# mindspore-lab/minddet

Hardware: AMD Instinct MI355X
Metric: images/sec, Faster R-CNN R50-FPN inference, COCO-shaped 1333x800 (padded 800x1344) (higher is better)
Workload: dtype bf16; 1 GPU; faster_rcnn_r50_fpn_800x1344 (BASELINE.json configs[2]); batch_per_gpu=120, streams=2, global_batch=120, parallelism=dp1 (image sharding + all_gather of detections), weights=random init, seed 7

## Files before the change

### minddet_amd/graphs.py

```python
import math
import os

import numpy as np
import torch

from . import det_ops, nn_ops
from .registry import BACKBONES, DETECTORS, HEADS, NECKS, READERS, ROI_HEAD, build_backbone, build_head, build_neck, build_roi_head


RPN_OVERLAP = os.environ.get("MD_RPN_OVERLAP", "1") == "1"
FUSE_BLOCKS = os.environ.get("MD_FUSE_BLOCKS", "1") == "1"
FUSE_DUAL = os.environ.get("MD_FUSE_DUAL", "1") == "1"
RPN_FUSED_HEAD = os.environ.get("MD_RPN_FUSED", "1") == "1"


class SplitForward:

    def __init__(self, model, streams=2):
        self.model, self.n = model, int(streams)
        self._streams = None
        self._primed = set()

    def __call__(self, images, prepare=None, **kw):
        ins = images if isinstance(images, (tuple, list)) else (images,)
        B = ins[0].shape[0]
        if self.n <= 1 or B < self.n or B % self.n or kw.get("return_aux"):
            return self.model.forward(images if prepare is None else prepare(*ins), **kw)
        dev = ins[0].device
        if self._streams is None or self._streams[0].device != dev:
            self._streams = [torch.cuda.Stream(device=dev) for _ in range(self.n)]
            self._primed = set()
        step = B // self.n

        def part(i):
            p = [t[i * step:(i + 1) * step] for t in ins]
            return p[0] if prepare is None else prepare(*p)

        cur = torch.cuda.current_stream(dev)
        key = (Module.generation, step, prepare is not None) + tuple(ins[0].shape[1:])
        if key not in self._primed:
            self.model.forward(part(0), **kw)
            self._primed.add(key)
        outs = []
        for i, st in enumerate(self._streams):
            st.wait_stream(cur)
            with torch.cuda.stream(st):
                outs.append(self.model.forward(part(i), **kw))
        for st in self._streams:
            cur.wait_stream(st)
        res = []
        for k in range(len(outs[0])):
            ts = [o[k] for o in outs]
            for t in ts:
                t.record_stream(cur)
            res.append(torch.cat(ts, 0))
        return tuple(res)


def _split_forward_of(model, test_cfg):
    model.streams = int((test_cfg or {}).get("streams", 1))
    model.forward_split = SplitForward(model, model.streams)


class ParamInit:

    def __init__(self, seed=7):
        self.rng = np.random.default_rng(seed)

    def conv(self, cout, cin, k, std=None):
        std = math.sqrt(2.0 / (k * k * cout)) if std is None else std
        return torch.from_numpy(self.rng.normal(0.0, std, (cout, cin, k, k)).astype(np.float32))

    def bn(self, c, eps=1e-5):
        return (torch.ones(c), torch.zeros(c), torch.from_numpy(self.rng.normal(0, 0.1, c).astype(np.float32)),
                torch.from_numpy(self.rng.uniform(0.5, 1.5, c).astype(np.float32)), eps)

    def bias(self, c, value=None, std=0.01):
        if value is not None:
            return torch.full((c,), float(value))
        return torch.from_numpy(self.rng.normal(0, std, c).astype(np.float32))


class Module:
    generation = 0

    def children(self):
        return []

    def modules(self):
        ch = self.children()
        return [m for c in ch for m in c.modules()] if ch else [self]

    conv_modules = modules

    def to(self, device):
        for c in self.children():
            c.to(device)
        self._derive(device)
        self._consts = {}
        Module.generation += 1
        return self

    def _derive(self, device):
        pass

    def const(self, key, build):
        if key not in self._consts:
            self._consts[key] = build()
        return self._consts[key]


def _segments(B, n, device):
    return torch.arange(0, (B + 1) * n, n, dtype=torch.int32, device=device)


def _image_hw(images):
    border = nn_ops.STEM_PAD_LO + nn_ops.STEM_PAD_HI if images.shape[3] == 4 else 0
    return images.shape[1] - border, images.shape[2] - border


class ConvModule(Module):

    def __init__(self, init, cin, cout, k, stride=1, pad=0, bn=True, relu=True, bias=False, bn_eps=1e-5, std=None,
                 bias_value=None, act=None):
        self.act = act if act is not None else ("relu" if relu else None)
        relu = self.act == "relu"
        self.cin, self.cout, self.k, self.stride, self.pad, self.relu = cin, cout, k, stride, pad, relu
        self.weight = init.conv(cout, cin, k, std)
        self.bn = init.bn(cout, bn_eps) if bn else None
        self.bias = init.bias(cout, bias_value) if bias else None
        self.packed = None

    def _derive(self, device):
        self.packed = nn_ops.pack_conv(self.weight, bias=self.bias, bn=self.bn, stride=self.stride, pad=self.pad,
                                       relu=self.act).to(device)

    def __call__(self, x, residual=None, out=None, c_off=0, x_c_off=None, res_c_off=None):
        return nn_ops.conv2d(x, self.packed, residual=residual, out=out, c_off=c_off, x_c_off=x_c_off, res_c_off=res_c_off)

    def macs(self, ho, wo):
        return ho * wo * self.cout * self.cin * self.k * self.k


def merged_conv(mods, device):
    m0 = mods[0]
    if any((m.cin, m.k, m.stride, m.pad, m.act, m.bn is None, m.bias is None) != (m0.cin, m0.k, m0.stride, m0.pad, m0.act, m0.bn is None, m0.bias is None)
           for m in mods):
        raise ValueError("merged_conv: the convs must share input, geometry and activation")
    w = torch.cat([m.weight for m in mods], 0)
    bn = None if m0.bn is None else tuple(torch.cat([torch.as_tensor(m.bn[i]) for m in mods]) for i in range(4)) + (m0.bn[4],)
    bias = None if m0.bias is None else torch.cat([m.bias for m in mods])
    return nn_ops.pack_conv(w, bias=bias, bn=bn, stride=m0.stride, pad=m0.pad, relu=m0.act).to(device)


class BasicBlock(Module):
    expansion = 1

    def __init__(self, init, inplanes, planes, stride=1, downsample=None):
        self.conv1 = ConvModule(init, inplanes, planes, 3, stride, 1)
        self.conv2 = ConvModule(init, planes, planes, 3, 1, 1, relu=True)
        self.downsample = downsample

    def children(self):
        return [self.conv1, self.conv2] + ([self.downsample] if self.downsample else [])

    def __call__(self, x):
        residual = self.downsample(x) if self.downsample is not None else x
        out = self.conv1(x)
        return self.conv2(out, residual=residual)


class Bottleneck(Module):
    expansion = 4

    def __init__(self, init, inplanes, planes, stride=1, downsample=None):
        self.conv1 = ConvModule(init, inplanes, planes, 1)
        self.conv2 = ConvModule(init, planes, planes, 3, stride, 1)
        self.conv3 = ConvModule(init, planes, planes * 4, 1, relu=True)
        self.downsample = downsample
        self._fused = self._dual = None

    def children(self):
        return [self.conv1, self.conv2, self.conv3] + ([self.downsample] if self.downsample else [])

    def _derive(self, device):
        pd = self.downsample.packed if self.downsample is not None else None
        self._fused = nn_ops.pack_bottleneck(self.conv1.packed, self.conv2.packed, self.conv3.packed, pd)
        self._dual = nn_ops.pack_dual(self.conv3.packed, pd) if pd is not None else None

    def __call__(self, x):
        if FUSE_BLOCKS and self._fused is not None:
            res = self.downsample(x) if (self.downsample is not None and self._fused.wd is None) else None
            return nn_ops.bottleneck(x, self._fused, residual=res)
        if FUSE_DUAL and self._dual is not None:
            return nn_ops.conv1x1_dual(self.conv2(self.conv1(x)), x, self._dual)
        residual = self.downsample(x) if self.downsample is not None else x
        return self.conv3(self.conv2(self.conv1(x)), residual=residual)


@BACKBONES.register_module
class ResNet(Module):
    SETTINGS = {18: (BasicBlock, [2, 2, 2, 2]), 34: (BasicBlock, [3, 4, 6, 3]), 50: (Bottleneck, [3, 4, 6, 3]),
                101: (Bottleneck, [3, 4, 23, 3])}

    def __init__(self, depth=50, base_width=64, seed=7, init=None, layers=None):
        block, default_layers = self.SETTINGS[depth]
        layers = layers or default_layers
        init = init or ParamInit(seed)
        self.block, self.inplanes = block, base_width
        self.conv1 = ConvModule(init, 3, base_width, 7, 2, 3)
        self.stages = []
        for i, n in enumerate(layers):
            self.stages.append(self._make_layer(init, block, base_width * (2 ** i), n, 1 if i == 0 else 2))
        self.out_channels = [base_width * (2 ** i) * block.expansion for i in range(4)]

    def _make_layer(self, init, block, planes, blocks, stride):
        downsample = None
        if stride != 1 or self.inplanes != planes * block.expansion:
            downsample = ConvModule(init, self.inplanes, planes * block.expansion, 1, stride, 0, relu=False)
        layers = [block(init, self.inplanes, planes, stride, downsample)]
        self.inplanes = planes * block.expansion
        for _ in range(1, blocks):
            layers.append(block(init, self.inplanes, planes))
        return layers

    def children(self):
        return [self.conv1] + [b for st in self.stages for b in st]

    def _derive(self, device):
        self.stem = None
        if self.conv1.cout == 64 and self.conv1.relu:
            self.stem = nn_ops.pack_stem(self.conv1.weight, bn=self.conv1.bn, bias=self.conv1.bias).to(device)

    def __call__(self, x):
        if x.shape[3] == 4:
            if self.stem is None:
                raise nn_ops._lib.MindDetHipError("ResNet: stem-layout input needs the 64-channel ReLU stem")
            x = nn_ops.stem_pool(x, self.stem)
        else:
            x = self.conv1(x)
            x = nn_ops.maxpool2d(x, 3, 2, 1, zero_pad=True)
        outs = []
        for st in self.stages:
            for b in st:
                x = b(x)
            outs.append(x)
        return tuple(outs)


@NECKS.register_module
class FPN(Module):

    def __init__(self, in_channels, out_channels=256, num_outs=5, seed=11, init=None):
        init = init or ParamInit(seed)
        self.lateral = [ConvModule(init, c, out_channels, 1, bn=False, relu=False, bias=True) for c in in_channels]
        self.output = [ConvModule(init, out_channels, out_channels, 3, 1, 1, bn=False, relu=False, bias=True)
                       for _ in in_channels]
        self.num_outs = num_outs

    def children(self):
        return self.lateral + self.output

    def __call__(self, feats):
        lats = [None] * len(feats)
        lats[-1] = self.lateral[-1](feats[-1])
        for i in range(len(feats) - 2, -1, -1):
            h, w = feats[i].shape[1], feats[i].shape[2]
            top = lats[i + 1]
            if top.shape[1] == (h + 1) // 2 and top.shape[2] == (w + 1) // 2:
                lats[i] = nn_ops.conv2d(feats[i], self.lateral[i].packed, residual=top, res_upsample=True)
            else:
                lats[i] = nn_ops.upsample_add(self.lateral[i](feats[i]), top)
        outs = [o(l) for o, l in zip(self.output, lats)]
        while len(outs) < self.num_outs:
            outs.append(nn_ops.maxpool2d(outs[-1], 1, 2, 0, zero_pad=False))
        return outs


@HEADS.register_module
class RPNHead(Module):

    def __init__(self, in_channels=256, feat_channels=256, strides=(4, 8, 16, 32, 64), scale=8.0,
                 ratios=(0.5, 1.0, 2.0), nms_pre=1000, max_per_img=1000, nms_thr=0.7, seed=13, init=None):
        init = init or ParamInit(seed)
        self.A = len(ratios)
        self.conv = ConvModule(init, in_channels, feat_channels, 3, 1, 1, bn=False, relu=True, bias=True, std=0.01)
        self.out = ConvModule(init, feat_channels, 5 * self.A, 1, bn=False, relu=False, bias=True, std=0.01)
        self.strides, self.scale, self.ratios = tuple(strides), scale, tuple(ratios)
        self.nms_pre, self.max_per_img, self.nms_thr = nms_pre, max_per_img, nms_thr

    def children(self):
        return [self.conv, self.out]

    def _static(self, feats, img_hw):
        B, dev = feats[0].shape[0], feats[0].device
        sizes = tuple((f.shape[1], f.shape[2]) for f in feats)

        def build():
            anchors = det_ops.fpn_anchors(sizes, self.strides, self.scale, self.ratios, device=dev)
            per, offs, o = [], [], 0
            for (h, w) in sizes:
                n = h * w * self.A
                per.append(anchors[o:o + n])
                offs.append(_segments(B, n, dev))
                o += n
            return dict(anchors=per, seg=offs, merged_seg=_segments(B, len(sizes) * self.nms_pre, dev))

        return self.const((B, sizes, img_hw), build)

    def __call__(self, feats, img_hw):
        st = self._static(feats, img_hw)
        B, L, k, A = feats[0].shape[0], len(feats), self.nms_pre, self.A
        dev = feats[0].device
        boxes = torch.empty((L, B, k, 4), dtype=torch.float32, device=dev)
        scores = torch.empty((L, B, k), dtype=torch.float32, device=dev)
        counts = torch.empty((L, B), dtype=torch.int32, device=dev)
        heads = []
        main = torch.cuda.current_stream(dev) if RPN_OVERLAP else None
        side = self.const("side", lambda: torch.cuda.Stream(dev)) if RPN_OVERLAP else None
        keep_alive = []
        if RPN_OVERLAP:
            for t in (boxes, scores, counts):
                t.record_stream(side)
        try:
            for l, f in enumerate(feats):
                if RPN_FUSED_HEAD and self.conv.cout == 256 and self.out.packed.cout == 16 and self.conv.relu:
                    head = nn_ops.conv2d_head(f, self.conv.packed, self.out.packed)
                else:
                    head = self.out(self.conv(f))
                heads.append(head)

                def select(l=l, f=f, head=head):
                    logits = nn_ops.slice_cast(head, 0, A)
                    _, idx, cnt = det_ops.topk_segmented(logits, st["seg"][l], k, out_cnt=counts[l],
                                                         max_segment=f.shape[1] * f.shape[2] * A)
                    det_ops.rpn_decode(head, st["anchors"][l], idx, cnt, A, img_hw, out_boxes=boxes[l], out_scores=scores[l])
                    keep_alive.append((logits, idx, cnt))

                if RPN_OVERLAP:
                    head.record_stream(side)
                    ev = torch.cuda.Event()
                    ev.record(main)
                    with torch.cuda.stream(side):
                        side.wait_event(ev)
                        select()
                else:
                    select()
        finally:
            if RPN_OVERLAP:
                main.wait_stream(side)
        keep, _, _ = det_ops.nms_aligned(boxes.view(L * B, k, 4), self.nms_thr, mode=det_ops.NMS_MODE_STRICT,
                                         count=counts.view(-1))
        mboxes, mscores = det_ops.rpn_merge(boxes, scores, keep.view(L, B, k))
        topv, topi, cnt = det_ops.topk_segmented(mscores, st["merged_seg"], self.max_per_img, max_segment=L * k)
        rois, roi_scores = det_ops.make_rois(mboxes, topv, topi, cnt)
        return rois, roi_scores, cnt, dict(heads=heads, boxes=boxes, scores=scores, counts=counts, keep=keep,
                                           mboxes=mboxes, mscores=mscores)


@ROI_HEAD.register_module
class StandardRoIHead(Module):

    def __init__(self, in_channels=256, fc_channels=1024, num_classes=80, roi_size=7, sampling_ratio=2,
                 featmap_strides=(4, 8, 16, 32), score_thr=0.05, nms_thr=0.5, max_per_img=100, nms_pre=2048,
                 seed=17, init=None):
        init = init or ParamInit(seed)
        self.nc, self.P, self.C = num_classes, roi_size, in_channels
        k_in = in_channels * roi_size * roi_size
        self.fc1 = ConvModule(init, k_in, fc_channels, 1, bn=False, relu=True, bias=True, std=math.sqrt(2.0 / k_in))
        self.fc2 = ConvModule(init, fc_channels, fc_channels, 1, bn=False, relu=True, bias=True,
                              std=math.sqrt(2.0 / fc_channels))
        self.reg_offset = (num_classes + 1 + 7) // 8 * 8
        n_out = self.reg_offset + 4 * num_classes
        self.fc_out = ConvModule(init, fc_channels, n_out, 1, bn=False, relu=False, bias=True, std=0.01)
        self.fc_out.weight[num_classes + 1:self.reg_offset] = 0
        self.fc_out.bias[num_classes + 1:self.reg_offset] = 0
        self.fc_out.weight[:num_classes + 1] *= 20.0
        self.strides, self.sampling = tuple(featmap_strides), sampling_ratio
        self.score_thr, self.nms_thr, self.max_per_img, self.nms_pre = score_thr, nms_thr, max_per_img, nms_pre
        self.prefix_status = det_ops.PrefixStatus()

    def children(self):
        return [self.fc1, self.fc2, self.fc_out]

    def __call__(self, feats, rois, roi_cnt, img_hw):
        B = feats[0].shape[0]
        R = rois.shape[0]
        post = R // B
        dev = rois.device
        pooled = det_ops.roi_align(list(feats[:len(self.strides)]), rois, self.P, [1.0 / s for s in self.strides],
                                   self.sampling, True)
        x = nn_ops.linear(pooled.view(R, self.P * self.P * self.C), self.fc1.packed)
        x = nn_ops.linear(x, self.fc2.packed)
        cls_reg = nn_ops.linear(x, self.fc_out.packed)
        cand = det_ops.rcnn_scores(cls_reg, roi_cnt, self.nc, self.score_thr)
        seg = self.const((B, post), lambda: _segments(B, post * self.nc, dev))
        sv, si, sc = det_ops.topk_segmented(cand, seg, self.nms_pre, max_segment=post * self.nc)
        boxes, labels = det_ops.rcnn_decode_selected(cls_reg, rois, si, sc, self.nc, self.reg_offset, img_hw)
        keep, kidx, num = det_ops.nms_aligned(boxes, self.nms_thr, mode=det_ops.NMS_MODE_STRICT, count=sc, group=labels,
                                              max_output=self.max_per_img)
        dets, count = det_ops.pack_detections(boxes, sv, labels, kidx, num, self.max_per_img, sel_cnt=sc,
                                              status=self.prefix_status.tensor(B, dev))
        return dets, count, dict(pooled=pooled, cls_reg=cls_reg, cand=cand, sel_scores=sv, sel_idx=si, sel_cnt=sc,
                                 boxes=boxes, labels=labels, keep=keep)


@DETECTORS.register_module
class FasterRCNN(Module):

    def __init__(self, backbone, neck, rpn_head, roi_head, train_cfg=None, test_cfg=None):
        self.backbone = build_backbone(backbone)
        neck = dict(neck)
        neck.setdefault("in_channels", self.backbone.out_channels)
        self.neck = build_neck(neck)
        self.rpn_head = build_head(rpn_head)
        self.roi_head = build_roi_head(roi_head)
        self.test_cfg = test_cfg
        _split_forward_of(self, test_cfg)

    def children(self):
        return [self.backbone, self.neck, self.rpn_head, self.roi_head]

    @property
    def prefix_status(self):
        return self.roi_head.prefix_status

    def extract_feat(self, images):
        return self.neck(self.backbone(images))

    def forward(self, images, return_aux=False):
        img_hw = _image_hw(images)
        feats = self.extract_feat(images)
        rois, roi_scores, roi_cnt, aux_rpn = self.rpn_head(feats, img_hw)
        dets, count, aux_roi = self.roi_head(feats, rois, roi_cnt, img_hw)
        if return_aux:
            return dets, count, dict(feats=feats, rois=rois, roi_scores=roi_scores, roi_cnt=roi_cnt, rpn=aux_rpn, roi=aux_roi)
        return dets, count

    __call__ = forward

    def macs_per_image(self, h, w, num_rois=None):
        total, hh, ww = 0, h, w
        bb = self.backbone

        def out_hw(m, hh, ww):
            return (hh + 2 * m.pad - m.k) // m.stride + 1, (ww + 2 * m.pad - m.k) // m.stride + 1

        hh, ww = out_hw(bb.conv1, hh, ww)
        total += bb.conv1.macs(hh, ww)
        hh, ww = (hh + 2 - 3) // 2 + 1, (ww + 2 - 3) // 2 + 1
        sizes = []
        for st in bb.stages:
            for b in st:
                h_in, w_in = hh, ww
                for m in b.modules():
                    if m is b.downsample:
                        ho, wo = out_hw(m, h_in, w_in)
                        total += m.macs(ho, wo)
                    else:
                        hh, ww = out_hw(m, hh, ww)
                        total += m.macs(hh, ww)
            sizes.append((hh, ww))
        for l, (a, b_) in zip(self.neck.lateral, sizes):
            total += l.macs(a, b_)
        for o, (a, b_) in zip(self.neck.output, sizes):
            total += o.macs(a, b_)
        lv = list(sizes)
        while len(lv) < self.neck.num_outs:
            lv.append(((lv[-1][0] - 1) // 2 + 1, (lv[-1][1] - 1) // 2 + 1))
        for (a, b_) in lv:
            total += self.rpn_head.conv.macs(a, b_) + self.rpn_head.out.macs(a, b_)
        r = num_rois if num_rois is not None else self.rpn_head.max_per_img
        for m in self.roi_head.modules():
            total += r * m.cout * m.cin
        return total


class DeconvModule(Module):

    def __init__(self, init, cin, cout, k, stride, pad, bn=True, relu=True, bn_eps=1e-5):
        self.cin, self.cout, self.k, self.stride, self.pad, self.relu = cin, cout, k, stride, pad, relu
        std = math.sqrt(2.0 / (k * k * cout))
        self.weight_t = torch.from_numpy(init.rng.normal(0.0, std, (cin, cout, k, k)).astype(np.float32))
        self.bn = init.bn(cout, bn_eps) if bn else None
        self.packed = None

    def _derive(self, device):
        self.packed = nn_ops.pack_conv_transpose(self.weight_t, bn=self.bn, stride=self.stride, pad=self.pad,
                                                 relu=self.relu).to(device)

    def __call__(self, x, out=None, c_off=0):
        return nn_ops.conv_transpose2d(x, self.packed, out=out, c_off=c_off)


@ROI_HEAD.register_module
class FCNMaskHead(Module):

    def __init__(self, in_channels=256, conv_channels=256, num_convs=4, num_classes=80, roi_size=14, sampling_ratio=2,
                 featmap_strides=(4, 8, 16, 32), seed=19, init=None):
        init = init or ParamInit(seed)
        self.nc, self.P, self.C = num_classes, roi_size, in_channels
        self.convs = []
        cin = in_channels
        for _ in range(num_convs):
            self.convs.append(ConvModule(init, cin, conv_channels, 3, 1, 1, bn=False, relu=True, bias=True))
            cin = conv_channels
        self.upsample = DeconvModule(init, cin, conv_channels, 2, 2, 0, bn=False, relu=True)
        self.logits = ConvModule(init, conv_channels, num_classes, 1, bn=False, relu=False, bias=True, std=0.05)
        self.strides, self.sampling = tuple(featmap_strides), sampling_ratio

    def children(self):
        return self.convs + [self.upsample, self.logits]

    def __call__(self, feats, dets):
        B, D = dets.shape[0], dets.shape[1]
        rois = det_ops.dets_to_rois(dets)
        x = det_ops.roi_align(list(feats[:len(self.strides)]), rois, self.P, [1.0 / s for s in self.strides], self.sampling, True)
        for m in self.convs:
            x = m(x)
        x = self.logits(self.upsample(x))
        masks = det_ops.mask_select(x, dets.view(B * D, 6), self.nc)
        return masks.view(B, D, 2 * self.P, 2 * self.P), dict(rois=rois, logits=x)


@DETECTORS.register_module
class MaskRCNN(FasterRCNN):

    def __init__(self, backbone, neck, rpn_head, roi_head, mask_head, train_cfg=None, test_cfg=None):
        super().__init__(backbone, neck, rpn_head, roi_head, train_cfg, test_cfg)
        self.mask_head = build_roi_head(mask_head)
        tc = test_cfg or {}
        self.paste = bool(tc.get("paste_masks", False))
        self.mask_thr = float(tc.get("mask_thr_binary", 0.5))

    def children(self):
        return super().children() + [self.mask_head]

    def forward(self, images, return_aux=False, paste=None):
        dets, count, aux = FasterRCNN.forward(self, images, return_aux=True)
        masks, aux_mask = self.mask_head(aux["feats"], dets)
        out = (dets, count, masks)
        if self.paste if paste is None else paste:
            out = out + (det_ops.paste_masks(masks, dets, _image_hw(images), self.mask_thr, bits=True),)
        if return_aux:
            aux["mask"] = aux_mask
            return out + (aux,)
        return out

# ... 808 lines not shown
```

### minddet_amd/nn_ops.py

```python
import ctypes

import torch

from . import _lib


class ConvTune(ctypes.Structure):
    _fields_ = [("chunk_limit", ctypes.c_int32), ("stream_rounds", ctypes.c_int32), ("stream_wgs_per_cu", ctypes.c_int32),
                ("stream_cache_bits", ctypes.c_int32), ("pers_min_k", ctypes.c_int32), ("dual_pp_min_k", ctypes.c_int32)]


class _ConvAttrs(ctypes.Structure):
    _fields_ = [("kh", ctypes.c_int32), ("kw", ctypes.c_int32), ("stride", ctypes.c_int32), ("pad", ctypes.c_int32),
                ("relu", ctypes.c_int32), ("variant", ctypes.c_int32), ("adv", ctypes.c_int32), ("pad_top", ctypes.c_int32),
                ("pad_left", ctypes.c_int32), ("sub_h", ctypes.c_int32), ("sub_w", ctypes.c_int32),
                ("out_stride", ctypes.c_int32), ("out_off_y", ctypes.c_int32), ("out_off_x", ctypes.c_int32),
                ("c_off", ctypes.c_int32), ("cout", ctypes.c_int32), ("res_upsample", ctypes.c_int32), ("korder", ctypes.c_int32),
                ("x_c_off", ctypes.c_int32), ("x_cin", ctypes.c_int32), ("res_slice", ctypes.c_int32), ("res_c_off", ctypes.c_int32),
                ("reserved0", ctypes.c_int32), ("tune", ConvTune)]


def cout_tile(cout):
    return 128 if cout > 64 else (64 if cout > 32 else 32)


def _round_up(x, m):
    return (x + m - 1) // m * m


KORDER_DEFAULT = 0


ACT_CODES = {None: 0, False: 0, True: 1, "relu": 1, "silu": 2, 0: 0, 1: 1, 2: 2}


class _PackedWB:

    def to(self, device):
        self.w, self.bias = self.w.to(device), self.bias.to(device)
        return self


class PackedConv(_PackedWB):

    def __init__(self, w, bias, cin, cout, kh, kw, stride, pad, relu):
        self.w, self.bias = w, bias
        self.cin, self.cout, self.kh, self.kw = cin, cout, kh, kw
        self.stride, self.pad, self.relu = stride, pad, relu

    def flops(self, n, ho, wo):
        return 2 * n * ho * wo * self.cout * self.cin_real * self.kh * self.kw

    cin_real = 0


def _fold_bn(weight, bias, bn):
    weight = weight.detach().to(torch.float32)
    if bn is None:
        return weight, (bias.detach().to(torch.float32) if bias is not None else torch.zeros(weight.shape[0]))
    gamma, beta, mean, var, eps = bn
    scale = gamma.to(torch.float32) / torch.sqrt(var.to(torch.float32) + eps)
    b = beta.to(torch.float32) - mean.to(torch.float32) * scale
    if bias is not None:
        b = b + bias.to(torch.float32) * scale
    return weight * scale.view(-1, 1, 1, 1), b


def pack_conv(weight, bias=None, bn=None, stride=1, pad=0, relu=False, cin_pad_to=8, cout_pad_to=8, korder=None):
    cout, cin, kh, kw = weight.shape
    weight, b = _fold_bn(weight, bias, bn)
    cin_p = _round_up(cin, cin_pad_to)
    cout_o = _round_up(cout, cout_pad_to)
    cout_p = _round_up(cout_o, cout_tile(cout_o))
    k_real = kh * kw * cin_p
    k_pad = _round_up(k_real, 64)
    wp = torch.zeros((cout_p, kh, kw, cin_p), dtype=torch.float32, device=weight.device)
    wp[:cout, :, :, :cin] = weight.permute(0, 2, 3, 1)
    if korder is None:
        halo = kh == 3 and kw == 3 and stride == 1 and pad == 1 and cin_p % 64 == 0 and cout_o >= 64
        korder = 1 if halo else KORDER_DEFAULT
    if korder == 1:
        wp = wp.reshape(cout_p, kh, kw, cin_p // 64, 64).permute(0, 3, 1, 2, 4).contiguous()
    wk = torch.zeros((cout_p, k_pad), dtype=torch.float32, device=weight.device)
    wk[:, :k_real] = wp.reshape(cout_p, k_real)
    bp = torch.zeros((cout_p,), dtype=torch.float32, device=weight.device)
    bp[:cout] = b.to(weight.device)
    pc = PackedConv(wk.to(torch.bfloat16).contiguous(), bp.contiguous(), cin_p, cout_o, kh, kw, stride, pad, ACT_CODES[relu])
    pc.cin_real = cin
    pc.korder = korder
    return pc


def conv_out_hw(h, w, pc):
    return (h + 2 * pc.pad - pc.kh) // pc.stride + 1, (w + 2 * pc.pad - pc.kw) // pc.stride + 1


import os as _os
TUNE = ConvTune(dual_pp_min_k=int(_os.environ.get("MD_DUAL_PP_MIN_K", "0")), pers_min_k=int(_os.environ.get("MD_PERS_MIN_K", "0")))


def conv2d(x, pc, residual=None, relu=None, out=None, variant=None, c_off=0, res_upsample=False, x_c_off=None, res_c_off=None, tune=None):
    n, h, w, c = x.shape
    if x_c_off is None and c != pc.cin:
        raise _lib.MindDetHipError(f"conv2d: input has {c} channels, layer packed for {pc.cin}")
    ho, wo = conv_out_hw(h, w, pc)
    if out is None:
        out = torch.empty((n, ho, wo, pc.cout), dtype=torch.bfloat16, device=x.device)
    attrs = _ConvAttrs(pc.kh, pc.kw, pc.stride, pc.pad, int(pc.relu if relu is None else relu),
                       int(variant or 0))
    attrs.korder = getattr(pc, "korder", 0)
    attrs.tune = TUNE if tune is None else tune
    attrs.res_upsample = int(bool(res_upsample))
    if x_c_off is not None:
        attrs.x_c_off, attrs.x_cin = int(x_c_off), pc.cin
    if res_c_off is not None:
        attrs.res_slice, attrs.res_c_off = 1, int(res_c_off)
    if out.shape[3] != pc.cout or c_off:
        attrs.adv, attrs.pad_top, attrs.pad_left, attrs.sub_h, attrs.sub_w = 1, pc.pad, pc.pad, ho, wo
        attrs.out_stride, attrs.c_off, attrs.cout = 1, int(c_off), pc.cout
    _lib.call("md_conv2d", [x, pc.w, pc.bias, residual, out], extra=attrs)
    return out


def conv2d_head(x, pc, pc2, variant=None, tune=None):
    n, h, w, c = x.shape
    if c != pc.cin or pc.cout != 256 or pc2.cin != 256 or pc2.cout != 16 or pc2.kh != 1 or pc2.stride != 1 or pc2.pad != 0:
        raise _lib.MindDetHipError("conv2d_head: needs a 256-channel conv followed by a 1x1 conv with 16 (padded) output channels")
    ho, wo = conv_out_hw(h, w, pc)
    y2 = torch.empty((n, ho, wo, 16), dtype=torch.bfloat16, device=x.device)
    attrs = _ConvAttrs(pc.kh, pc.kw, pc.stride, pc.pad, 1, int(variant or 0))
    attrs.korder = getattr(pc, "korder", 0)
    attrs.tune = TUNE if tune is None else tune
    _lib.call("md_conv2d_head", [x, pc.w, pc.bias, pc2.w, pc2.bias, y2], extra=attrs)
    return y2


class PackedBottleneck:

    def __init__(self, pc1, pc2, pc3, pd=None):
        self.cin, self.cout = pc1.cin, pc3.cout
        self.w1, self.w2, self.w3 = pc1.w, pc2.w, pc3.w
        self.b12 = torch.cat([pc1.bias[:64], pc2.bias[:64]]).contiguous()
        self.b3 = pc3.bias
        self.wd, self.bd = (pd.w, pd.bias) if pd is not None else (None, None)
        self.macs_per_pixel = pc1.cin_real * 64 + 9 * 64 * 64 + 64 * 256 + (pd.cin_real * 256 if pd is not None else 0)

    def flops_bytes(self, n, h, w, with_residual_tensor=False):
        px = n * h * w
        wts = self.w1.numel() + self.w2.numel() + self.w3.numel() + (self.wd.numel() if self.wd is not None else 0)
        byts = 2.0 * (px * (self.cin + 256 + (256 if with_residual_tensor else 0)) + wts)
        return 2.0 * px * self.macs_per_pixel, byts


def pack_bottleneck(pc1, pc2, pc3, pd=None):
    ok = (pc1.kh == 1 and pc1.stride == 1 and pc1.pad == 0 and pc1.relu == 1 and pc1.cout == 64 and pc1.cin in (64, 256) and
          tuple(pc1.w.shape) == (64, pc1.cin) and
          pc2.kh == 3 and pc2.kw == 3 and pc2.stride == 1 and pc2.pad == 1 and pc2.relu == 1 and pc2.cin == 64 and pc2.cout == 64 and
          tuple(pc2.w.shape) == (64, 576) and
          pc3.kh == 1 and pc3.stride == 1 and pc3.pad == 0 and pc3.relu == 1 and pc3.cin == 64 and pc3.cout == 256 and
          tuple(pc3.w.shape) == (256, 64))
    if not ok:
        return None
    fuse_ds = (pd is not None and pd.kh == 1 and pd.stride == 1 and pd.pad == 0 and pd.relu == 0 and pd.cin == 64 and pc1.cin == 64 and
               pd.cout == 256 and tuple(pd.w.shape) == (256, 64))
    return PackedBottleneck(pc1, pc2, pc3, pd if fuse_ds else None)


def bottleneck(x, blk, residual=None, out=None, tune=None):
    n, h, w, c = x.shape
    if c != blk.cin:
        raise _lib.MindDetHipError(f"bottleneck: input has {c} channels, block packed for {blk.cin}")
    if out is None:
        out = torch.empty((n, h, w, 256), dtype=torch.bfloat16, device=x.device)
    fused_ds = blk.wd is not None and residual is None
    _lib.call("md_bottleneck", [x, blk.w1, blk.b12, blk.w2, blk.w3, blk.b3, residual, blk.wd if fused_ds else None,
                                blk.bd if fused_ds else None, out], extra=tune)
    return out


class _C3PairAttrs(ctypes.Structure):
    _fields_ = [("x_c_off", ctypes.c_int32), ("y_c_off", ctypes.c_int32), ("shortcut", ctypes.c_int32), ("pass_through", ctypes.c_int32)]


class PackedC3Pair:

    def __init__(self, pc1, pc2):
        self.c = pc1.cin
        self.w1, self.w2 = pc1.w, pc2.w
        self.b12 = torch.cat([pc1.bias[:self.c], pc2.bias[:self.c]]).contiguous()
        self.macs_per_pixel = pc1.cin_real * self.c + 9 * pc2.cin_real * self.c

    def flops_bytes(self, n, h, w, shortcut=True):
        px = n * h * w
        return 2.0 * px * self.macs_per_pixel, 2.0 * (px * 2 * self.c + self.w1.numel() + self.w2.numel())


def pack_c3_pair(pc1, pc2):
    c = pc1.cin
    k1, k2 = _round_up(c, 64), _round_up(9 * c, 64)
    ok = (c in (32, 64, 128) and pc1.kh == 1 and pc1.stride == 1 and pc1.pad == 0 and pc1.relu == 2 and pc1.cout == c and tuple(pc1.w.shape) == (c, k1) and
          pc2.kh == 3 and pc2.kw == 3 and pc2.stride == 1 and pc2.pad == 1 and pc2.relu == 2 and pc2.cin == c and pc2.cout == c and
          tuple(pc2.w.shape) == (c, k2) and getattr(pc2, "korder", 0) == (0 if c == 32 else 1))
    return PackedC3Pair(pc1, pc2) if ok else None


def c3_pair(x, pk, out, x_c_off=0, y_c_off=0, shortcut=True, pass_through=False):
    _lib.call("md_c3_pair", [x, pk.w1, pk.b12, pk.w2, out], extra=_C3PairAttrs(int(x_c_off), int(y_c_off), int(bool(shortcut)), int(bool(pass_through))))
    return out


class _DualAttrs(ctypes.Structure):
    _fields_ = [("stride_b", ctypes.c_int32), ("relu", ctypes.c_int32), ("tune", ConvTune)]


class PackedDual:

    def __init__(self, pc3, pd):
        self.ca, self.cb, self.cout, self.stride, self.relu = pc3.cin, pd.cin, pc3.cout, pd.stride, int(pc3.relu)
        self.w = torch.cat([pc3.w[:, :pc3.cin], pd.w[:, :pd.cin]], dim=1).contiguous()
        self.bias = (pc3.bias + pd.bias).contiguous()
        self.cin_real = pc3.cin_real + pd.cin_real

    def flops_bytes(self, n, ho, wo):
        px = n * ho * wo
        return 2.0 * px * self.cout * (self.ca + self.cb), 2.0 * (px * (self.ca + self.cb + self.cout) + self.w.numel())


def pack_dual(pc3, pd):
    ok = (pc3.kh == 1 and pc3.stride == 1 and pc3.pad == 0 and pc3.relu in (0, 1) and pd.kh == 1 and pd.pad == 0 and pd.relu == 0 and
          pc3.cout == pd.cout and pc3.cout > 64 and pc3.cin % 64 == 0 and pd.cin % 64 == 0 and cout_tile(pc3.cout) == 128 and
          tuple(pc3.w.shape) == (pd.w.shape[0], pc3.cin) and pd.w.shape[1] == pd.cin)
    return PackedDual(pc3, pd) if ok else None


def conv1x1_dual(xa, xb, pk, out=None, tune=None):
    n, ho, wo, ca = xa.shape
    if ca != pk.ca or xb.shape[3] != pk.cb:
        raise _lib.MindDetHipError(f"conv1x1_dual: inputs have {ca} / {xb.shape[3]} channels, packed for {pk.ca} / {pk.cb}")
    if out is None:
        out = torch.empty((n, ho, wo, pk.cout), dtype=torch.bfloat16, device=xa.device)
    _lib.call("md_conv1x1_dual", [xa, xb, pk.w, pk.bias, None, out], extra=_DualAttrs(int(pk.stride), int(pk.relu), TUNE if tune is None else tune))
    return out


class PackedConvT:

    def __init__(self, subs, cin, cout, k, stride, relu):
        self.subs, self.cin, self.cout, self.k, self.stride, self.relu = subs, cin, cout, k, stride, relu

    def to(self, device):
        for pc, _ in self.subs:
            pc.to(device)
        return self


def pack_conv_transpose(weight_t, bias=None, bn=None, stride=2, pad=1, relu=False):
    cin, cout, k, k2 = weight_t.shape
    s = stride
    if not (k == k2 and ((k == 4 and s == 2 and pad == 1) or (k == s and pad == 0))):
        raise _lib.MindDetHipError("pack_conv_transpose: unsupported (kernel, stride, padding)")
    subs = []
    for py in range(s):
        for px in range(s):
            kys = [ky for ky in range(k) if (ky - py - pad) % s == 0]
            kxs = [kx for kx in range(k) if (kx - px - pad) % s == 0]
            dys = sorted(((py + pad - ky) // s, ky) for ky in kys)
            dxs = sorted(((px + pad - kx) // s, kx) for kx in kxs)
            w_sub = torch.stack([torch.stack([weight_t[:, :, ky, kx] for _, kx in dxs], -1) for _, ky in dys], -2)
            pc = pack_conv(w_sub.permute(1, 0, 2, 3).contiguous(), bias=bias, bn=bn, stride=1, pad=0, relu=relu)
            subs.append((pc, dict(py=py, px=px, pad_top=-dys[0][0], pad_left=-dxs[0][0])))
    return PackedConvT(subs, cin, cout, k, s, relu)


def conv_transpose2d(x, pct, out=None, c_off=0):
    n, h, w, c = x.shape
    s = pct.stride
    c_out = pct.subs[0][0].cout
    if out is None:
        out = torch.empty((n, h * s, w * s, c_out), dtype=torch.bfloat16, device=x.device)
    for pc, m in pct.subs:
        attrs = _ConvAttrs(pc.kh, pc.kw, 1, 0, int(pct.relu), 0)
        attrs.adv, attrs.pad_top, attrs.pad_left, attrs.sub_h, attrs.sub_w = 1, m["pad_top"], m["pad_left"], h, w
        attrs.out_stride, attrs.out_off_y, attrs.out_off_x, attrs.c_off, attrs.cout = s, m["py"], m["px"], int(c_off), pc.cout
        attrs.korder = getattr(pc, "korder", 0)
        attrs.tune = TUNE
        _lib.call("md_conv2d", [x, pc.w, pc.bias, None, out], extra=attrs)
    return out


def linear(x2d, pc, relu=None):
    r, c = x2d.shape
    y = conv2d(x2d.view(r, 1, 1, c), pc, relu=relu)
    return y.view(r, pc.cout)


class _PoolAttrs(ctypes.Structure):
    _fields_ = [("k", ctypes.c_int32), ("stride", ctypes.c_int32), ("pad", ctypes.c_int32), ("zero_pad", ctypes.c_int32)]


class _SliceAttrs(ctypes.Structure):
    _fields_ = [("c0", ctypes.c_int32), ("width", ctypes.c_int32)]


def maxpool2d(x, k=3, stride=2, pad=1, zero_pad=True):
    n, h, w, c = x.shape
    ho, wo = (h + 2 * pad - k) // stride + 1, (w + 2 * pad - k) // stride + 1
    y = torch.empty((n, ho, wo, c), dtype=torch.bfloat16, device=x.device)
    _lib.call("md_maxpool2d", [x, y], extra=_PoolAttrs(k, stride, pad, int(zero_pad)))
    return y


class _SppfAttrs(ctypes.Structure):
    _fields_ = [("channels", ctypes.c_int32), ("k", ctypes.c_int32)]


def sppf_pool_fits(h, w, c):
    return _lib.lib().md_sppf_pool_groups(int(h), int(w), int(c)) > 0


def sppf_pool(buf, c, k=5):
    _lib.call("md_sppf_pool", [buf], extra=_SppfAttrs(int(c), int(k)))
    return buf


def upsample_add(lateral, top):
    y = torch.empty_like(lateral)
    _lib.call("md_upsample_add", [lateral, top, y])
    return y


def slice_cast(x, c0, width):
    y = torch.empty(tuple(x.shape[:-1]) + (width,), dtype=torch.float32, device=x.device)
    _lib.call("md_slice_cast", [x, y], extra=_SliceAttrs(c0, width))
    return y


def nhwc_to_nchw_f32(x, c0, width):
    n, h, w, _ = x.shape
    y = torch.empty((n, width, h, w), dtype=torch.float32, device=x.device)
    _lib.call("md_nhwc_to_nchw_f32", [x, y], extra=_SliceAttrs(c0, width))
    return y


def concat_copy(src, dst, c0):
    _lib.call("md_concat_copy", [src, dst], extra=_SliceAttrs(int(c0), src.shape[3]))
    return dst


class _Upsample2xAttrs(ctypes.Structure):
    _fields_ = [("c0", ctypes.c_int32), ("width", ctypes.c_int32), ("src_c0", ctypes.c_int32)]


def upsample2x(src, dst=None, c0=0, src_c0=0, width=None):
    n, h, w, cs = src.shape
    c = cs - src_c0 if width is None else width
    if dst is None:
        dst = torch.empty((n, 2 * h, 2 * w, c), dtype=torch.bfloat16, device=src.device)
    _lib.call("md_upsample2x", [src, dst], extra=_Upsample2xAttrs(int(c0), int(c), int(src_c0)))
    return dst


STEM_PAD_LO, STEM_PAD_HI = 7, 9


class PackedStem(_PackedWB):
    def __init__(self, w, bias):
        self.w, self.bias = w, bias


def pack_stem(weight, bn=None, bias=None):
    cout, cin, kh, kw = weight.shape
    if (cout, kh, kw) != (64, 7, 7) or cin > 3:
        raise _lib.MindDetHipError("pack_stem: expects a [64, <=3, 7, 7] stem convolution")
    weight, b = _fold_bn(weight, bias, bn)
    wp = torch.zeros((64, 7, 8, 4), dtype=torch.float32)
    wp[:, :, :7, :cin] = weight.permute(0, 2, 3, 1)
    return PackedStem(wp.reshape(64, 224).to(torch.bfloat16).contiguous(), b.contiguous())


class _StemConvAttrs(ctypes.Structure):
    _fields_ = [("kh", ctypes.c_int32), ("act", ctypes.c_int32)]


class PackedStemConv(_PackedWB):
    def __init__(self, w, bias, kh, act, cout):
        self.w, self.bias, self.kh, self.act, self.cout = w, bias, kh, act, cout


def pack_stem_conv(weight, bn=None, bias=None, act=None):
    cout, cin, kh, kw = weight.shape
    if kh != kw or kh not in (6, 3) or cin > 3 or cout not in (32, 64):
        return None
    weight, b = _fold_bn(weight, bias, bn)
    kx, x0 = (8, 1) if kh == 6 else (4, 0)
    wp = torch.zeros((cout, kh, kx, 4), dtype=torch.float32)
    wp[:, :, x0:x0 + kw, :cin] = weight.permute(0, 2, 3, 1)
    return PackedStemConv(wp.reshape(cout, kh * kx * 4).to(torch.bfloat16).contiguous(), b.contiguous(), kh, ACT_CODES[act], cout)


def stem_conv(x4, ps):
    n, hp, wp, c = x4.shape
    h, w = hp - STEM_PAD_LO - STEM_PAD_HI, wp - STEM_PAD_LO - STEM_PAD_HI
    y = torch.empty((n, h // 2, w // 2, ps.cout), dtype=torch.bfloat16, device=x4.device)
    _lib.call("md_stem_conv", [x4, ps.w, ps.bias, y], extra=_StemConvAttrs(ps.kh, ps.act))
    return y


def stem_layout_ok(h, w):
    return h % 16 == 0 and w % 64 == 0


def to_stem_layout(x):
    n, h, w, _ = x.shape
    out = torch.zeros((n, h + STEM_PAD_LO + STEM_PAD_HI, w + STEM_PAD_LO + STEM_PAD_HI, 4), dtype=torch.bfloat16, device=x.device)
    out[:, STEM_PAD_LO:STEM_PAD_LO + h, STEM_PAD_LO:STEM_PAD_LO + w, :3] = x[..., :3]
    return out


def stem_pool(x4, ps):
    n, hp, wp, c = x4.shape
    h, w = hp - STEM_PAD_LO - STEM_PAD_HI, wp - STEM_PAD_LO - STEM_PAD_HI
    y = torch.empty((n, h // 4, w // 4, 64), dtype=torch.bfloat16, device=x4.device)
    _lib.call("md_stem_pool", [x4, ps.w, ps.bias, y])
    return y


class _PoolAttrs3(ctypes.Structure):
    _fields_ = [("k", ctypes.c_int32), ("stride", ctypes.c_int32), ("pad", ctypes.c_int32), ("zero_pad", ctypes.c_int32)]


def deform_conv2d(x, pc_offset, pc, relu=None):
    n, h, w, c = x.shape
    if getattr(pc, "korder", 0) != 0 or pc.kh != pc.kw or pc.cin != c:
        raise _lib.MindDetHipError("deform_conv2d: the main conv must be packed with korder=0 for this input")
    off = conv2d(x, pc_offset)
    ho, wo = off.shape[1], off.shape[2]
    cols = torch.empty((n, ho, wo, pc.kh * pc.kw * c), dtype=torch.bfloat16, device=x.device)
    _lib.call("md_deform_cols", [x, off, cols], extra=_PoolAttrs3(pc.kh, pc.stride, pc.pad, 0))
    pw = PackedConv(pc.w, pc.bias, pc.kh * pc.kw * c, pc.cout, 1, 1, 1, 0, pc.relu)
    pw.cin_real, pw.korder = pc.kh * pc.kw * c, 0
    return conv2d(cols, pw, relu=relu)


class _PreAttrs(ctypes.Structure):
    _fields_ = [("out_h", ctypes.c_int32), ("out_w", ctypes.c_int32), ("pad_lo", ctypes.c_int32), ("pad_hi", ctypes.c_int32)]


def image_preprocess(img_u8, mat, mean, std, out_hw, stem_layout=True):
    n = img_u8.shape[0]
    ho, wo = out_hw
    lo, hi, c = (STEM_PAD_LO, STEM_PAD_HI, 4) if stem_layout else (0, 0, 8)
    out = torch.empty((n, ho + lo + hi, wo + lo + hi, c), dtype=torch.bfloat16, device=img_u8.device)
    norm = torch.tensor(list(mean) + list(std), dtype=torch.float32, device=img_u8.device)
    _lib.call("md_image_preprocess", [img_u8, mat, norm, out], extra=_PreAttrs(ho, wo, lo, hi))
    return out


GROUPED_MAX_GROUPS = 64


class _GroupedAttrs(ctypes.Structure):
    _fields_ = [("k", ctypes.c_int32), ("relu", ctypes.c_int32), ("groups", ctypes.c_int32), ("cin_g", ctypes.c_int32),
                ("x_c_off", ctypes.c_int32), ("reserved0", ctypes.c_int32), ("cout", ctypes.c_int32 * GROUPED_MAX_GROUPS),
                ("y_off", ctypes.c_int32 * GROUPED_MAX_GROUPS), ("w_row", ctypes.c_int32 * GROUPED_MAX_GROUPS)]


class PackedGrouped(_PackedWB):

    def __init__(self, w, bias, k, couts, w_rows, y_offs, relu):
        self.w, self.bias, self.k, self.relu = w, bias, k, relu
        self.couts, self.w_rows, self.y_offs = list(couts), list(w_rows), list(y_offs)
        self.groups, self.cin_g = len(self.couts), 64

    def flops(self, n, h, w):
        return 2 * n * h * w * sum(self.couts) * self.cin_g * self.k * self.k

    def attrs(self, x_c_off=0):
        at = _GroupedAttrs(self.k, int(self.relu), self.groups, self.cin_g, int(x_c_off), 0)
        for g in range(self.groups):
            at.cout[g], at.y_off[g], at.w_row[g] = self.couts[g], self.y_offs[g], self.w_rows[g]
        return at


def pack_conv2d_grouped(convs, y_offs=None, relu=False):
    if not 1 <= len(convs) <= GROUPED_MAX_GROUPS:
        raise _lib.MindDetHipError(f"pack_conv2d_grouped: 1..{GROUPED_MAX_GROUPS} groups, got {len(convs)}")
    k = convs[0][0].shape[2]
    ws, bs, couts = [], [], []
    for weight, bias, bn in convs:
        c, cin, kh, kw = weight.shape
        if cin != 64 or kh != k or kw != k or k not in (1, 3) or not 1 <= c <= 16:
            raise _lib.MindDetHipError(f"pack_conv2d_grouped: every group is a [1..16, 64, k, k] conv with one k in (1, 3), got {tuple(weight.shape)}")
        pc = pack_conv(weight, bias=bias, bn=bn, pad=k // 2, korder=0)
        ws.append(pc.w[:c, :k * k * 64])
        bs.append(pc.bias[:c])
        couts.append(c)
    w_rows = [sum(couts[:g]) for g in range(len(couts))]
    if y_offs is None:
        y_offs = w_rows
    return PackedGrouped(torch.cat(ws).contiguous(), torch.cat(bs).contiguous(), k, couts, w_rows, y_offs, int(bool(relu)))


def conv2d_grouped(x, pk, out, x_c_off=0):
    _lib.call("md_conv2d_grouped", [x, pk.w, pk.bias, out], extra=pk.attrs(x_c_off))
    return out
```

Before: 2183 images/sec.

## Fuse block conv3 with next block's conv1 in a pointwise chain kernel

Adds a HIP kernel that computes a bottleneck's final 1x1 conv (128->512) with bias, residual add and ReLU, then immediately runs the next block's first 1x1 conv (512->128) with ReLU on the tile still held in LDS. The goal is to avoid re-reading the 512-channel activation from global memory and to save one kernel launch per chained block pair. It applies only to stage blocks not already covered by the fully fused bottleneck path, and only at 128/512 channel widths. The kernel uses a deep DMA ring and 512-thread single-block-per-CU launch, which may limit occupancy.

```diff
diff --git a/include/minddet_hip_chain.h b/include/minddet_hip_chain.h
--- /dev/null
+++ b/include/minddet_hip_chain.h
@@ -0,0 +1,15 @@
+#ifndef MINDDET_HIP_CHAIN_H_
+#define MINDDET_HIP_CHAIN_H_
+
+#include "minddet_hip.h"
+
+#ifdef __cplusplus
+extern "C" {
+#endif
+
+int md_pw_chain(MD_AOT_ARGS);
+
+#ifdef __cplusplus
+}
+#endif
+#endif
diff --git a/minddet_amd/csrc/pwchain.hip b/minddet_amd/csrc/pwchain.hip
--- /dev/null
+++ b/minddet_amd/csrc/pwchain.hip
@@ -0,0 +1,279 @@
+#include <hip/hip_runtime.h>
+#include <stdint.h>
+
+#include "aot.h"
+#include "device.h"
+#include "../../include/minddet_hip_chain.h"
+
+namespace md {
+
+struct ChainArgs {
+    const uint16_t *t2, *res, *w3, *w1;
+    const float *b3, *b1;
+    uint16_t *y, *t1;
+    long long M;
+    int n_tiles;
+};
+
+#define MD_CHAIN_WAIT_VMCNT(N) asm volatile("s_waitcnt vmcnt(%0)" ::"n"(N) : "memory")
+
+constexpr int PC_PT = 32;
+constexpr int PC_NR = 4, PC_D = PC_NR - 1;
+constexpr int PC_SLOT = PC_PT * 256;
+constexpr int PC_EW = PC_PT * 128;
+constexpr int PC_NE = PC_EW / 1024;
+constexpr int PC_SET = 8 * PC_EW;
+constexpr int PC_T1 = PC_PT * 256;
+constexpr int PC_OFF_Y = PC_NR * PC_SLOT, PC_OFF_T1 = PC_OFF_Y + 2 * PC_SET, PC_OFF_BIAS = PC_OFF_T1 + PC_T1;
+constexpr int PC_LDS = PC_OFF_BIAS + 512 * 4;
+constexpr int PC_PER_ITER = 1 + 1 + 2 * PC_NE;
+
+__global__ __launch_bounds__(512, 1) void pw_chain_kernel(ChainArgs a) {
+    typedef __attribute__((address_space(3))) void lds_void;
+    extern __shared__ __attribute__((aligned(16))) char smem[];
+    char *ring = smem;
+    const int tid = threadIdx.x, lane = tid & 63;
+    const int wave = __builtin_amdgcn_readfirstlane(tid >> 6);
+    const int lr = lane & 31, lh = lane >> 5;
+    const int p16 = lane & 15, q = lane >> 4;
+    char *Y = smem + PC_OFF_Y + wave * PC_EW;
+    char *T1 = smem + PC_OFF_T1;
+    float *bias_lds = reinterpret_cast<float *>(smem + PC_OFF_BIAS);
+
+    const int G = gridDim.x, per = a.n_tiles / G, extra = a.n_tiles % G, g = blockIdx.x;
+    const int t0 = g * per + (g < extra ? g : extra);
+    const int nt = per + (g < extra ? 1 : 0);
+    const int cout_w = wave * 64;
+
+    const int xrow = wave * 4 + (lane >> 4);
+    const unsigned xoff = (unsigned)(xrow * 256 + (((lane & 15) ^ (xrow & 15)) << 4));
+    unsigned eoff[PC_NE];
+#pragma unroll
+    for (int i = 0; i < PC_NE; ++i) {
+        const int row = i * 8 + (lane >> 3), lc = (lane & 7) ^ ((row >> 1) & 7);
+        eoff[i] = (unsigned)(row * 1024 + lc * 16);
+    }
+    int foff[8];
+#pragma unroll
+    for (int s = 0; s < 8; ++s) foff[s] = lr * 256 + (((2 * s + lh) ^ (lr & 15)) << 4);
+    const int eswz = (lr >> 1) & 7;
+    int g2off[2];
+#pragma unroll
+    for (int h = 0; h < 2; ++h) g2off[h] = p16 * 128 + (((h * 4 + q) ^ ((p16 >> 1) & 7)) << 4);
+    const int t1w = p16 * 256 + (((2 * wave + (q >> 1)) ^ p16) << 4) + (q & 1) * 8;
+    const int t1row = wave * 4 + (lane >> 4);
+    const unsigned t1off = (unsigned)(t1row * 256 + (((lane & 15) ^ (t1row & 15)) << 4));
+
+    auto clip = [](long long rem) { return (int)(rem > 0x7fffffffLL ? 0x7fffffffLL : (rem < 0 ? 0 : rem)); };
+    auto x_desc = [&](int t) {
+        const bool live = t < nt;
+        const long long m0 = live ? (long long)(t0 + t) * PC_PT : 0;
+        return srd(a.t2 + m0 * 128, clip(live ? (a.M - m0) * 256 : 0));
+    };
+    auto r_desc = [&](int t) {
+        const bool live = t < nt;
+        const long long m0 = live ? (long long)(t0 + t) * PC_PT : 0;
+        return srd(a.res + m0 * 512 + cout_w, clip(live ? (a.M - m0) * 1024 - cout_w * 2 : 0));
+    };
+    auto y_desc = [&](int t) {
+        const long long m0 = (long long)(t0 + t) * PC_PT;
+        return srd(a.y + m0 * 512 + cout_w, clip((a.M - m0) * 1024 - cout_w * 2));
+    };
+    auto t1_desc = [&](int t) {
+        const bool live = t >= 0;
+        const long long m0 = live ? (long long)(t0 + t) * PC_PT : 0;
+        return srd(a.t1 + m0 * 128, clip(live ? (a.M - m0) * 256 : 0));
+    };
+    auto dma_x = [&](int t, int slot) {
+        __amdgpu_buffer_rsrc_t rs = x_desc(t);
+        __builtin_amdgcn_raw_ptr_buffer_load_lds(rs, (lds_void *)(ring + slot * PC_SLOT + wave * 1024), 16, (int)xoff, 0, 0, 0);
+    };
+    auto dma_res = [&](int t, int set) {
+        __amdgpu_buffer_rsrc_t rs = r_desc(t);
+#pragma unroll
+        for (int i = 0; i < PC_NE; ++i)
+            __builtin_amdgcn_raw_ptr_buffer_load_lds(rs, (lds_void *)(Y + set * PC_SET + i * 1024), 16, (int)eoff[i], 0, 0, 0);
+    };
+
+#pragma unroll
+    for (int t = 0; t < PC_D; ++t) dma_x(t, t);
+    dma_res(0, 0);
+    bias_lds[tid] = a.b3[tid];
+    bf16x8 wr[2][8];
+#pragma unroll
+    for (int b = 0; b < 2; ++b)
+#pragma unroll
+        for (int s = 0; s < 8; ++s) wr[b][s] = *reinterpret_cast<const bf16x8 *>(a.w3 + (size_t)(cout_w + b * 32 + lr) * 128 + s * 16 + lh * 8);
+    bf16x8 w1r[16];
+#pragma unroll
+    for (int ks = 0; ks < 16; ++ks) w1r[ks] = *reinterpret_cast<const bf16x8 *>(a.w1 + (size_t)(wave * 16 + p16) * 512 + ks * 32 + q * 8);
+    const f32x4 b1v = *reinterpret_cast<const f32x4 *>(a.b1 + wave * 16 + q * 4);
+    asm volatile("s_waitcnt vmcnt(0)" ::: "memory");
+    __syncthreads();
+
+    int s_cur = 0, s_new = PC_D, set = 0;
+    for (int t = 0; t < nt; ++t) {
+        __builtin_amdgcn_sched_barrier(0);
+        MD_CHAIN_WAIT_VMCNT(PC_D * PC_PER_ITER - 1);
+        asm volatile("s_waitcnt lgkmcnt(0)" ::: "memory");
+        __builtin_amdgcn_s_barrier();
+        __builtin_amdgcn_sched_barrier(0);
+        dma_x(t + PC_D, s_new);
+        {
+            __amdgpu_buffer_rsrc_t rt = t1_desc(t - 1);
+            u32x4 v = *reinterpret_cast<const u32x4 *>(T1 + wave * 1024 + lane * 16);
+            MD_BUFFER_STORE_B128(v, rt, t1off, 0, 0);
+        }
+        __builtin_amdgcn_sched_barrier(0);
+        dma_res(t + 1, set ^ 1);
+        __builtin_amdgcn_sched_barrier(0);
+
+        const char *S = ring + s_cur * PC_SLOT;
+        f32x16 acc[2];
+#pragma unroll
+        for (int b = 0; b < 2; ++b)
+#pragma unroll
+            for (int e = 0; e < 16; ++e) acc[b][e] = 0.f;
+        bf16x8 fb[2];
+        fb[0] = *reinterpret_cast<const bf16x8 *>(S + foff[0]);
+#pragma unroll
+        for (int s = 0; s < 8; ++s) {
+            if (s + 1 < 8) fb[(s + 1) & 1] = *reinterpret_cast<const bf16x8 *>(S + foff[s + 1]);
+#pragma unroll
+            for (int b = 0; b < 2; ++b) acc[b] = __builtin_amdgcn_mfma_f32_32x32x16_bf16(wr[b][s], fb[s & 1], acc[b], 0, 0, 0);
+        }
+        s_cur = (s_cur + 1) & (PC_NR - 1);
+        s_new = (s_new + 1) & (PC_NR - 1);
+
+        char *E = Y + set * PC_SET;
+        u32x2 pk[2][4];
+#pragma unroll
+        for (int b = 0; b < 2; ++b) {
+            f32x4 bv[4];
+#pragma unroll
+            for (int gq = 0; gq < 4; ++gq) bv[gq] = *reinterpret_cast<const f32x4 *>(bias_lds + cout_w + b * 32 + 8 * gq + 4 * lh);
+            __builtin_amdgcn_sched_barrier(0);
+#pragma unroll
+            for (int gq = 0; gq < 4; ++gq) {
+                const f32x2 s01 = (f32x2){acc[b][4 * gq + 0], acc[b][4 * gq + 1]} + (f32x2){bv[gq].x, bv[gq].y};
+                const f32x2 s23 = (f32x2){acc[b][4 * gq + 2], acc[b][4 * gq + 3]} + (f32x2){bv[gq].z, bv[gq].w};
+                pk[b][gq].x = pk_bf16(s01.x, s01.y);
+                pk[b][gq].y = pk_bf16(s23.x, s23.y);
+            }
+        }
+        __builtin_amdgcn_sched_barrier(0);
+        MD_CHAIN_WAIT_VMCNT(PC_NE + 2 + PC_NE);
+        __builtin_amdgcn_sched_barrier(0);
+        u32x2 rv[2][4];
+#pragma unroll
+        for (int b = 0; b < 2; ++b)
+#pragma unroll
+            for (int gq = 0; gq < 4; ++gq) rv[b][gq] = *reinterpret_cast<const u32x2 *>(E + lr * 128 + (((4 * b + gq) ^ eswz) << 4) + 8 * lh);
+        __builtin_amdgcn_sched_barrier(0);
+#pragma unroll
+        for (int b = 0; b < 2; ++b)
+#pragma unroll
+            for (int gq = 0; gq < 4; ++gq) {
+                const f32x2 a01 = bf2f_pair(pk[b][gq].x) + bf2f_pair(rv[b][gq].x), a23 = bf2f_pair(pk[b][gq].y) + bf2f_pair(rv[b][gq].y);
+                u32x2 o;
+                o.x = pk_relu_bf16(pk_bf16(a01.x, a01.y));
+                o.y = pk_relu_bf16(pk_bf16(a23.x, a23.y));
+                *reinterpret_cast<u32x2 *>(E + lr * 128 + (((4 * b + gq) ^ eswz) << 4) + 8 * lh) = o;
+            }
+        __amdgpu_buffer_rsrc_t ry = y_desc(t);
+        MD_WAVE_LDS_ORDER();
+#pragma unroll
+        for (int i = 0; i < PC_NE; ++i) {
+            u32x4 v = *reinterpret_cast<const u32x4 *>(E + i * 1024 + lane * 16);
+            MD_BUFFER_STORE_B128(v, ry, eoff[i], 0, 0);
+        }
+
+        __builtin_amdgcn_sched_barrier(0);
+        asm volatile("s_waitcnt lgkmcnt(0)" ::: "memory");
+        __builtin_amdgcn_s_barrier();
+        __builtin_amdgcn_sched_barrier(0);
+        const char *YT = smem + PC_OFF_Y + set * PC_SET;
+        f32x4 c2[2];
+#pragma unroll
+        for (int pb = 0; pb < 2; ++pb) c2[pb] = (f32x4){0.f, 0.f, 0.f, 0.f};
+        auto y_frag = [&](int ks, int pb) { return *reinterpret_cast<const bf16x8 *>(YT + (ks >> 1) * PC_EW + pb * 2048 + g2off[ks & 1]); };
+        bf16x8 yb[2][2][2];
+#pragma unroll
+        for (int k2 = 0; k2 < 2; ++k2)
+#pragma unroll
+            for (int pb = 0; pb < 2; ++pb) yb[0][k2][pb] = y_frag(k2, pb);
+#pragma unroll
+        for (int kg = 0; kg < 8; ++kg) {
+            if (kg + 1 < 8) {
+#pragma unroll
+                for (int k2 = 0; k2 < 2; ++k2)
+#pragma unroll
+                    for (int pb = 0; pb < 2; ++pb) yb[(kg + 1) & 1][k2][pb] = y_frag(2 * (kg + 1) + k2, pb);
+            }
+            __builtin_amdgcn_sched_barrier(0);
+#pragma unroll
+            for (int k2 = 0; k2 < 2; ++k2)
+#pragma unroll
+                for (int pb = 0; pb < 2; ++pb)
+                    c2[pb] = __builtin_amdgcn_mfma_f32_16x16x32_bf16(w1r[2 * kg + k2], yb[kg & 1][k2][pb], c2[pb], 0, 0, 0);
+            __builtin_amdgcn_sched_barrier(0);
+        }
+#pragma unroll
+        for (int pb = 0; pb < 2; ++pb) {
+            const f32x4 v = c2[pb] + b1v;
+            u32x2 pk;
+            pk.x = pk_relu_bf16(pk_bf16(v.x, v.y));
+            pk.y = pk_relu_bf16(pk_bf16(v.z, v.w));
+            *reinterpret_cast<u32x2 *>(T1 + pb * 4096 + t1w) = pk;
+        }
+        set ^= 1;
+    }
+    __builtin_amdgcn_sched_barrier(0);
+    asm volatile("s_waitcnt lgkmcnt(0)" ::: "memory");
+    __builtin_amdgcn_s_barrier();
+    __builtin_amdgcn_sched_barrier(0);
+    {
+        __amdgpu_buffer_rsrc_t rt = t1_desc(nt - 1);
+        u32x4 v = *reinterpret_cast<const u32x4 *>(T1 + wave * 1024 + lane * 16);
+        MD_BUFFER_STORE_B128(v, rt, t1off, 0, 0);
+    }
+}
+
+static bool ranges_overlap(const void *p, long long pn, const void *r, long long rn) {
+    const char *pb = (const char *)p, *rb = (const char *)r;
+    return pb < rb + rn && rb < pb + pn;
+}
+
+}
+
+using namespace md;
+
+extern "C" int md_pw_chain(MD_AOT_ARGS) {
+    Args g(MD_ARGS, 8, 8);
+    g.tensor(0, BF16, 4); g.tensor(1, BF16, 4); g.tensor(2, BF16, 2); g.tensor(3, F32, 1); g.tensor(4, BF16, 2); g.tensor(5, F32, 1);
+    g.tensor(6, BF16, 4); g.tensor(7, BF16, 4);
+    const int64_t N = g.d(0, 0), H = g.d(0, 1), W = g.d(0, 2);
+    g.require(g.d(0, 3) == 128 && g.d(1, 3) == 512 && g.d(6, 3) == 512 && g.d(7, 3) == 128);
+    g.require(g.d(2, 0) == 512 && g.d(2, 1) == 128 && g.d(3, 0) == 512 && g.d(4, 0) == 128 && g.d(4, 1) == 512 && g.d(5, 0) == 128);
+    for (int i : {1, 6, 7}) g.require(g.d(i, 0) == N && g.d(i, 1) == H && g.d(i, 2) == W);
+    g.require(N >= 0 && H >= 0 && W >= 0);
+    if (int rc = g.rc()) return rc;
+    if (N * H * W == 0) return MD_OK;
+    if (!g.have({0, 1, 2, 3, 4, 5, 6, 7})) return MD_ERR_ARG;
+    if (!fits_i32(N) || !fits_i32(H) || !fits_i32(W) || !fits_i32(N * H) || !fits_i32(N * H * W)) return MD_ERR_SIZE;
+    const long long M = N * H * W;
+    const long long nb[8] = {M * 256, M * 1024, 0, 0, 0, 0, M * 1024, M * 256};
+    for (int o : {6, 7})
+        for (int i : {0, 1})
+            if (ranges_overlap(params[o], nb[o], params[i], nb[i])) return MD_ERR_ARG;
+    if (ranges_overlap(params[6], nb[6], params[7], nb[7])) return MD_ERR_ARG;
+    ChainArgs a;
+    a.t2 = (const uint16_t *)params[0]; a.res = (const uint16_t *)params[1]; a.w3 = (const uint16_t *)params[2]; a.b3 = (const float *)params[3];
+    a.w1 = (const uint16_t *)params[4]; a.b1 = (const float *)params[5]; a.y = (uint16_t *)params[6]; a.t1 = (uint16_t *)params[7];
+    a.M = M;
+    a.n_tiles = (int)((M + PC_PT - 1) / PC_PT);
+    if (ensure_dyn_lds((const void *)pw_chain_kernel, PC_LDS) != MD_OK) return MD_ERR_HIP;
+    const unsigned grid = a.n_tiles < 256 ? (unsigned)a.n_tiles : 256u;
+    hipLaunchKernelGGL(pw_chain_kernel, dim3(grid), dim3(512), PC_LDS, (hipStream_t)stream, a);
+    return launched();
+}
diff --git a/minddet_amd/graphs.py b/minddet_amd/graphs.py
--- a/minddet_amd/graphs.py
+++ b/minddet_amd/graphs.py
@@ -11,6 +11,7 @@
 RPN_OVERLAP = os.environ.get("MD_RPN_OVERLAP", "1") == "1"
 FUSE_BLOCKS = os.environ.get("MD_FUSE_BLOCKS", "1") == "1"
 FUSE_DUAL = os.environ.get("MD_FUSE_DUAL", "1") == "1"
+PW_CHAIN = os.environ.get("MD_PW_CHAIN", "1") == "1"
 RPN_FUSED_HEAD = os.environ.get("MD_RPN_FUSED", "1") == "1"
 
 
@@ -188,14 +189,18 @@
         self._fused = nn_ops.pack_bottleneck(self.conv1.packed, self.conv2.packed, self.conv3.packed, pd)
         self._dual = nn_ops.pack_dual(self.conv3.packed, pd) if pd is not None else None
 
-    def __call__(self, x):
-        if FUSE_BLOCKS and self._fused is not None:
-            res = self.downsample(x) if (self.downsample is not None and self._fused.wd is None) else None
-            return nn_ops.bottleneck(x, self._fused, residual=res)
-        if FUSE_DUAL and self._dual is not None:
-            return nn_ops.conv1x1_dual(self.conv2(self.conv1(x)), x, self._dual)
+    def __call__(self, x, t1=None, chain=None):
+        if t1 is None and chain is None:
+            if FUSE_BLOCKS and self._fused is not None:
+                res = self.downsample(x) if (self.downsample is not None and self._fused.wd is None) else None
+                return nn_ops.bottleneck(x, self._fused, residual=res)
+            if FUSE_DUAL and self._dual is not None:
+                return nn_ops.conv1x1_dual(self.conv2(self.conv1(x)), x, self._dual)
         residual = self.downsample(x) if self.downsample is not None else x
-        return self.conv3(self.conv2(self.conv1(x)), residual=residual)
+        t2 = self.conv2(self.conv1(x) if t1 is None else t1)
+        if chain is not None:
+            return nn_ops.pw_chain(t2, residual, chain)
+        return self.conv3(t2, residual=residual)
 
 
 @BACKBONES.register_module
@@ -231,6 +236,14 @@
         self.stem = None
         if self.conv1.cout == 64 and self.conv1.relu:
             self.stem = nn_ops.pack_stem(self.conv1.weight, bn=self.conv1.bn, bias=self.conv1.bias).to(device)
+        self._chains = {}
+        if self.block is Bottleneck:
+            for si, st in enumerate(self.stages):
+                for bi in range(1, len(st) - 1):
+                    if st[bi].downsample is None and st[bi + 1].downsample is None and st[bi]._fused is None and st[bi + 1]._fused is None:
+                        pk = nn_ops.pack_pw_chain(st[bi].conv3.packed, st[bi + 1].conv1.packed)
+                        if pk is not None:
+                            self._chains[(si, bi)] = pk
 
     def __call__(self, x):
         if x.shape[3] == 4:
@@ -241,9 +254,16 @@
             x = self.conv1(x)
             x = nn_ops.maxpool2d(x, 3, 2, 1, zero_pad=True)
         outs = []
-        for st in self.stages:
-            for b in st:
-                x = b(x)
+        for si, st in enumerate(self.stages):
+            t1 = None
+            for bi, b in enumerate(st):
+                chain = self._chains.get((si, bi)) if PW_CHAIN else None
+                if chain is not None:
+                    x, t1 = b(x, t1=t1, chain=chain)
+                elif t1 is not None:
+                    x, t1 = b(x, t1=t1), None
+                else:
+                    x = b(x)
             outs.append(x)
         return tuple(outs)
 
diff --git a/minddet_amd/nn_ops.py b/minddet_amd/nn_ops.py
--- a/minddet_amd/nn_ops.py
+++ b/minddet_amd/nn_ops.py
@@ -243,6 +243,34 @@
     return out
 
 
+class PackedPwChain:
+
+    def __init__(self, pc3, pc1):
+        self.w3, self.b3, self.w1, self.b1 = pc3.w, pc3.bias, pc1.w, pc1.bias
+        self.cin_real = pc3.cin_real
+
+    def flops_bytes(self, n, h, w):
+        px = n * h * w
+        return 2.0 * px * (512 * 128 + 128 * 512), 2.0 * (px * (128 + 512 + 512 + 128) + self.w3.numel() + self.w1.numel())
+
+
+def pack_pw_chain(pc3, pc1):
+    def plain1x1(pc, cin, cout):
+        return (pc.kh == 1 and pc.kw == 1 and pc.stride == 1 and pc.pad == 0 and pc.relu == 1 and pc.cin == cin and pc.cout == cout and
+                tuple(pc.w.shape) == (cout, cin) and tuple(pc.bias.shape) == (cout,))
+    return PackedPwChain(pc3, pc1) if plain1x1(pc3, 128, 512) and plain1x1(pc1, 512, 128) else None
+
+
+def pw_chain(t2, res, pk):
+    n, h, w, c = t2.shape
+    if c != 128 or tuple(res.shape) != (n, h, w, 512):
+        raise _lib.MindDetHipError(f"pw_chain: inputs are {tuple(t2.shape)} / {tuple(res.shape)}, need [N,H,W,128] / [N,H,W,512]")
+    y = torch.empty((n, h, w, 512), dtype=torch.bfloat16, device=t2.device)
+    t1 = torch.empty((n, h, w, 128), dtype=torch.bfloat16, device=t2.device)
+    _lib.call("md_pw_chain", [t2, res, pk.w3, pk.b3, pk.w1, pk.b1, y, t1])
+    return y, t1
+
+
 class PackedConvT:
 
     def __init__(self, subs, cin, cout, k, stride, relu):
```

Result: faster. 2217 images/sec (median of 6 runs) (+1.6%).
